# oneam/h264bsd

Hardware: AMD Instinct MI355X
Metric: 1080p macroblocks/s (higher is better)
Workload: dtype u8; 1 GPU; 256 concurrent copies of test_1920x1080.h264 per GPU (73 pictures x 8160 MB), kernel-only replay from HBM-resident frame jobs, inter+intra reconstruction + in-loop deblocking; streams_per_gpu=256, parallelism=streams/1, stream_groups=1, row_bands=library default (engine.hip TailConfig)

## Files before the change

h264bsd_amd/csrc/kernels/k_dbk.hip.h:

```cpp
#pragma once
namespace h264k {
#ifndef DBK_WGS
#define DBK_WGS 32
#endif
#ifndef DBK_WG_WAVES
#define DBK_WG_WAVES 4
#endif
__global__ __launch_bounds__(64 * DBK_WG_WAVES) void k_dbk(const FrameDesc *__restrict__ frames)
{
    __shared__ uint32_t s_tab[32 + 64];
    if (threadIdx.x < 64) {
        const uint32_t t = threadIdx.x, ok = t < 52;
        reinterpret_cast<uint8_t *>(s_tab)[t] = ok ? c_alpha[t] : 0;
        reinterpret_cast<uint8_t *>(s_tab)[64 + t] = ok ? c_beta[t] : 0;
        s_tab[32 + t] = ok ? (uint32_t)c_tc0[t][0] | ((uint32_t)c_tc0[t][1] << 8) | ((uint32_t)c_tc0[t][2] << 16) : 0u;
    }
    __syncthreads();
    const FrameDesc &fd = FD_REF(frames, blockIdx.y);
    const int m = threadIdx.x & 15;
    const int wmb = fd.wmb;
    const uint32_t n_dbk = fd.n_dbk;
    uint32_t di = blockIdx.x * (4 * DBK_WG_WAVES) + (threadIdx.x >> 4);
    const bool live0 = di < n_dbk;
    if (__ballot(live0) == 0ull) return;
    uint32_t mb = live0 ? fd.dbki[di] : 0u;
    bool live = live0;
  for (;;) {
    const uint32_t ndi = di + (4u * DBK_WG_WAVES) * gridDim.x;
    uint32_t nmb = mb;
    const bool nlive = live && ndi < n_dbk;
    if (nlive) nmb = fd.dbki[ndi];
    const uint32_t mbx = mb - mb_row(fd, mb) * (uint32_t)wmb;
    const uint32_t mbl = mbx ? mb - 1 : mb, mbt = mb >= (uint32_t)wmb ? mb - wmb : mb;
    FjMbRec q, pl, pt;
    const int dir = m >> 3, e = (m >> 1) & 3, kh = m & 1;
    int qx[2], qy[2], px[2], py[2];
    uint32_t mva[2], mvb[2];
#pragma unroll
    for (int kk = 0; kk < 2; kk++) {
        const int k = 2 * kh + kk;
        qx[kk] = dir ? k : e; qy[kk] = dir ? e : k;
        px[kk] = dir ? k : (e ? e - 1 : 3); py[kk] = dir ? (e ? e - 1 : 3) : k;
    }
    {
        const H264K_GLOBAL uint8_t *rq = (const H264K_GLOBAL uint8_t *)(fd.recs + mb), *rl = (const H264K_GLOBAL uint8_t *)(fd.recs + mbl),
                                   *rt = (const H264K_GLOBAL uint8_t *)(fd.recs + mbt);
        uint4 w[6] = { ld16g(rq), ld16g(rq + 16), ld16g(rl), ld16g(rl + 16), ld16g(rt), ld16g(rt + 16) };
#pragma unroll
        for (int i = 0; i < 6; i++) asm volatile("" : "+v"(w[i].x), "+v"(w[i].y), "+v"(w[i].z), "+v"(w[i].w));
        __builtin_memcpy(&q, &w[0], 32); __builtin_memcpy(&pl, &w[2], 32); __builtin_memcpy(&pt, &w[4], 32);
    }
    {
        const FjMbRec &pr = e ? q : (dir ? pt : pl);
        const bool q_one = (q.pred & FJ_PRED_UNIFORM_MV) || q.kind != FJ_MB_INTER, p_one = (pr.pred & FJ_PRED_UNIFORM_MV) || pr.kind != FJ_MB_INTER;
        const uint32_t q_mv = q.kind == FJ_MB_INTER ? (uint32_t)(uint16_t)q.mv[0] | ((uint32_t)(uint16_t)q.mv[1] << 16) : 0u;
        const uint32_t p_mv = pr.kind == FJ_MB_INTER ? (uint32_t)(uint16_t)pr.mv[0] | ((uint32_t)(uint16_t)pr.mv[1] << 16) : 0u;
#pragma unroll
        for (int kk = 0; kk < 2; kk++) {
            mva[kk] = q_mv; mvb[kk] = p_mv;
            if (!q_one) mva[kk] = *(const H264K_GLOBAL uint32_t *)(fd.mvx + 32 * (size_t)q.mvx + 2 * (4 * qy[kk] + qx[kk]));
            if (!p_one) mvb[kk] = *(const H264K_GLOBAL uint32_t *)(fd.mvx + 32 * (size_t)pr.mvx + 2 * (4 * py[kk] + px[kk]));
        }
    }
    uint8_t *out = fd.dbk + (size_t)mb * DBK_REC_BYTES;
    uint8_t *any_out = fd.dbk + (size_t)fd.n_mbs * DBK_REC_BYTES + mb;
    const bool filtered = live && q.dbk && q.kind != FJ_MB_ABSENT;
    if (live && !filtered && m == 0) { *reinterpret_cast<uint16_t *>(out + 46) = 0; *any_out = 0; }
    uint32_t bs2 = 0;
    const bool f_left = (q.dbk & FJ_DBK_LEFT) && mbx, f_top = (q.dbk & FJ_DBK_TOP) && mb >= (uint32_t)wmb;
    if (filtered) {
        const bool edge_on = e ? true : (dir ? f_top : f_left);
        if (edge_on) {
            const int p_kind = e ? q.kind : (dir ? pt.kind : pl.kind);
            const int parts = (q.pred >> FJ_PRED_PARTS_SHIFT) & 3;
            const uint32_t p_coded = e ? q.coded : (dir ? pt.coded : pl.coded);
            uint32_t qrefs, prefs, t0, t1;
            __builtin_memcpy(&qrefs, q.ref_slot, 4);
            __builtin_memcpy(&t0, pl.ref_slot, 4);
            __builtin_memcpy(&t1, pt.ref_slot, 4);
            prefs = e ? qrefs : (dir ? t1 : t0);
            const bool intra_edge = is_intra_kind(q.kind) || is_intra_kind(p_kind);
            const bool no_motion_edge = e && (parts == FJ_PARTS_16x16 || (parts == FJ_PARTS_16x8 && !(dir == 1 && e == 2)) || (parts == FJ_PARTS_8x16 && !(dir == 0 && e == 2)));
#pragma unroll
            for (int kk = 0; kk < 2; kk++) {
                int my_bs;
                if (intra_edge) my_bs = e ? 3 : 4;
                else if (((q.coded >> z_of(qx[kk], qy[kk])) & 1) || ((p_coded >> z_of(px[kk], py[kk])) & 1)) my_bs = 2;
                else if (no_motion_edge) my_bs = 0;
                else if (((qrefs >> (8 * ((qy[kk] >> 1) * 2 + (qx[kk] >> 1)))) & 255u) != ((prefs >> (8 * ((py[kk] >> 1) * 2 + (px[kk] >> 1)))) & 255u)) my_bs = 1;
                else {
                    const int ax = (int16_t)(mva[kk] & 0xFFFFu), ay = (int32_t)mva[kk] >> 16, bx2 = (int16_t)(mvb[kk] & 0xFFFFu), by2 = (int32_t)mvb[kk] >> 16;
                    my_bs = (abs(ax - bx2) >= 4 || abs(ay - by2) >= 4) ? 1 : 0;
                }
                bs2 |= (uint32_t)my_bs << (4 * kk);
            }
        }
    }
    uint32_t v = bs2;
    v |= (uint32_t)__builtin_amdgcn_update_dpp(0, (int)v, 0x101, 0xF, 0xF, true) << 8;
    v |= (uint32_t)__builtin_amdgcn_update_dpp(0, (int)v, 0x102, 0xF, 0xF, true) << 16;
    const unsigned long long bal = __ballot(bs2 != 0u);
    const uint32_t bal16 = (uint32_t)(bal >> (threadIdx.x & 48)) & 0xFFFFu;
    const bool any = bal16 != 0u;
    const uint32_t sched = (any ? DBKF_ANY : 0u) | ((bal16 & 0x0003u) ? DBKF_LEFT : 0u) | ((bal16 & 0x0300u) ? DBKF_TOP : 0u) |
                           ((bal16 & 0xFCFCu) ? DBKF_INNER : 0u);
    if (filtered) {
        if ((m & 3) == 0) *reinterpret_cast<uint32_t *>(out + m) = v;
        if (m < 6) {
            const int c = m;
            const int side = c % 3;
            const int pqp = side == 0 ? (int)pl.qp_y : side == 1 ? (int)pt.qp_y : (int)q.qp_y;
            int a = (int)q.qp_y, b = pqp;
            if (c >= 3) {
                a = qpc_of(clip3(0, 51, a + q.cqp_off));
                b = qpc_of(clip3(0, 51, b + q.cqp_off));
            }
            const int qpav = (a + b + 1) >> 1;
            const int ia = clip3(0, 51, qpav + q.alpha_off), ib = clip3(0, 51, qpav + q.beta_off);
            const uint32_t t = s_tab[32 + ia];
            *reinterpret_cast<uint32_t *>(out + 16 + 4 * c) = (uint32_t)reinterpret_cast<const uint8_t *>(s_tab)[ia] |
                ((uint32_t)reinterpret_cast<const uint8_t *>(s_tab)[64 + ib] << 8) | ((t & 0xFFFFu) << 16);
            out[40 + c] = (uint8_t)(t >> 16);
        }
        if (m == 12) {
            *reinterpret_cast<uint16_t *>(out + 46) = (uint16_t)((f_left ? FJ_DBK_LEFT : 0u) | (f_top ? FJ_DBK_TOP : 0u) | (q.dbk & FJ_DBK_INNER) | (any ? 0x100u : 0u));
            *any_out = (uint8_t)sched;
        }
    }
    if (__ballot(nlive) == 0ull) return;
    di = ndi; mb = nmb; live = nlive;
  }
}

}
```

Baseline: 1.782 billion macroblocks/s.

## Stage deblock MB records and output records through LDS with cooperative loads

Instead of every lane loading all three 32-byte macroblock records (current, left, top), six lanes per 16-lane group each load one 16-byte chunk into LDS. After a wave sync, each lane reads only the current record and the neighbour record it needs. The per-MB deblock output record is assembled in LDS and written back with three 16-byte stores in place of scattered 4-byte and byte stores. The default workgroup count per frame also doubles from 32 to 64. This cuts redundant global load traffic and VGPR pressure, at the cost of LDS use and extra wave syncs.

```diff
diff --git a/h264bsd_amd/csrc/kernels/k_dbk.hip.h b/h264bsd_amd/csrc/kernels/k_dbk.hip.h
--- a/h264bsd_amd/csrc/kernels/k_dbk.hip.h
+++ b/h264bsd_amd/csrc/kernels/k_dbk.hip.h
@@ -1,7 +1,7 @@
 #pragma once
 namespace h264k {
 #ifndef DBK_WGS
-#define DBK_WGS 32
+#define DBK_WGS 64
 #endif
 #ifndef DBK_WG_WAVES
 #define DBK_WG_WAVES 4
@@ -15,8 +15,12 @@
         reinterpret_cast<uint8_t *>(s_tab)[64 + t] = ok ? c_beta[t] : 0;
         s_tab[32 + t] = ok ? (uint32_t)c_tc0[t][0] | ((uint32_t)c_tc0[t][1] << 8) | ((uint32_t)c_tc0[t][2] << 16) : 0u;
     }
+    __shared__ u32x4 s_in[DBK_WG_WAVES][4][6];
+    __shared__ u32x4 s_out[DBK_WG_WAVES][4][3];
     __syncthreads();
     const FrameDesc &fd = FD_REF(frames, blockIdx.y);
+    H264K_LDS u32x4 *const in = (H264K_LDS u32x4 *)&s_in[threadIdx.x >> 6][(threadIdx.x >> 4) & 3][0];
+    H264K_LDS uint8_t *const rec = (H264K_LDS uint8_t *)&s_out[threadIdx.x >> 6][(threadIdx.x >> 4) & 3][0];
     const int m = threadIdx.x & 15;
     const int wmb = fd.wmb;
     const uint32_t n_dbk = fd.n_dbk;
@@ -32,7 +36,7 @@
     if (nlive) nmb = fd.dbki[ndi];
     const uint32_t mbx = mb - mb_row(fd, mb) * (uint32_t)wmb;
     const uint32_t mbl = mbx ? mb - 1 : mb, mbt = mb >= (uint32_t)wmb ? mb - wmb : mb;
-    FjMbRec q, pl, pt;
+    FjMbRec q, pr;
     const int dir = m >> 3, e = (m >> 1) & 3, kh = m & 1;
     int qx[2], qy[2], px[2], py[2];
     uint32_t mva[2], mvb[2];
@@ -42,16 +46,21 @@
         qx[kk] = dir ? k : e; qy[kk] = dir ? e : k;
         px[kk] = dir ? k : (e ? e - 1 : 3); py[kk] = dir ? (e ? e - 1 : 3) : k;
     }
+    const int side = m >= 3 ? m - 3 : m;
+    uint32_t pqp;
     {
-        const H264K_GLOBAL uint8_t *rq = (const H264K_GLOBAL uint8_t *)(fd.recs + mb), *rl = (const H264K_GLOBAL uint8_t *)(fd.recs + mbl),
-                                   *rt = (const H264K_GLOBAL uint8_t *)(fd.recs + mbt);
-        uint4 w[6] = { ld16g(rq), ld16g(rq + 16), ld16g(rl), ld16g(rl + 16), ld16g(rt), ld16g(rt + 16) };
-#pragma unroll
-        for (int i = 0; i < 6; i++) asm volatile("" : "+v"(w[i].x), "+v"(w[i].y), "+v"(w[i].z), "+v"(w[i].w));
-        __builtin_memcpy(&q, &w[0], 32); __builtin_memcpy(&pl, &w[2], 32); __builtin_memcpy(&pt, &w[4], 32);
+        if (m < 6) {
+            const uint32_t src = m < 2 ? mb : m < 4 ? mbl : mbt;
+            const uint4 w = ld16g((const H264K_GLOBAL uint8_t *)(fd.recs + src) + 16 * (m & 1));
+            in[m] = (u32x4){ w.x, w.y, w.z, w.w };
+        }
+        wave_sync();
+        const int pi = e ? 0 : dir ? 4 : 2;
+        const u32x4 w[4] = { in[0], in[1], in[pi], in[pi + 1] };
+        pqp = ((const H264K_LDS uint8_t *)(in + (side == 0 ? 2 : side == 1 ? 4 : 0)))[1];
+        __builtin_memcpy(&q, &w[0], 32); __builtin_memcpy(&pr, &w[2], 32);
     }
     {
-        const FjMbRec &pr = e ? q : (dir ? pt : pl);
         const bool q_one = (q.pred & FJ_PRED_UNIFORM_MV) || q.kind != FJ_MB_INTER, p_one = (pr.pred & FJ_PRED_UNIFORM_MV) || pr.kind != FJ_MB_INTER;
         const uint32_t q_mv = q.kind == FJ_MB_INTER ? (uint32_t)(uint16_t)q.mv[0] | ((uint32_t)(uint16_t)q.mv[1] << 16) : 0u;
         const uint32_t p_mv = pr.kind == FJ_MB_INTER ? (uint32_t)(uint16_t)pr.mv[0] | ((uint32_t)(uint16_t)pr.mv[1] << 16) : 0u;
@@ -62,23 +71,21 @@
             if (!p_one) mvb[kk] = *(const H264K_GLOBAL uint32_t *)(fd.mvx + 32 * (size_t)pr.mvx + 2 * (4 * py[kk] + px[kk]));
         }
     }
-    uint8_t *out = fd.dbk + (size_t)mb * DBK_REC_BYTES;
-    uint8_t *any_out = fd.dbk + (size_t)fd.n_mbs * DBK_REC_BYTES + mb;
+    H264K_GLOBAL uint8_t *out = (H264K_GLOBAL uint8_t *)fd.dbk + (size_t)mb * DBK_REC_BYTES;
+    H264K_GLOBAL uint8_t *any_out = (H264K_GLOBAL uint8_t *)fd.dbk + (size_t)fd.n_mbs * DBK_REC_BYTES + mb;
     const bool filtered = live && q.dbk && q.kind != FJ_MB_ABSENT;
-    if (live && !filtered && m == 0) { *reinterpret_cast<uint16_t *>(out + 46) = 0; *any_out = 0; }
+    if (live && !filtered && m == 0) *reinterpret_cast<H264K_GLOBAL uint16_t *>(out + 46) = 0;
     uint32_t bs2 = 0;
     const bool f_left = (q.dbk & FJ_DBK_LEFT) && mbx, f_top = (q.dbk & FJ_DBK_TOP) && mb >= (uint32_t)wmb;
     if (filtered) {
         const bool edge_on = e ? true : (dir ? f_top : f_left);
         if (edge_on) {
-            const int p_kind = e ? q.kind : (dir ? pt.kind : pl.kind);
+            const int p_kind = pr.kind;
             const int parts = (q.pred >> FJ_PRED_PARTS_SHIFT) & 3;
-            const uint32_t p_coded = e ? q.coded : (dir ? pt.coded : pl.coded);
-            uint32_t qrefs, prefs, t0, t1;
+            const uint32_t p_coded = pr.coded;
+            uint32_t qrefs, prefs;
             __builtin_memcpy(&qrefs, q.ref_slot, 4);
-            __builtin_memcpy(&t0, pl.ref_slot, 4);
-            __builtin_memcpy(&t1, pt.ref_slot, 4);
-            prefs = e ? qrefs : (dir ? t1 : t0);
+            __builtin_memcpy(&prefs, pr.ref_slot, 4);
             const bool intra_edge = is_intra_kind(q.kind) || is_intra_kind(p_kind);
             const bool no_motion_edge = e && (parts == FJ_PARTS_16x16 || (parts == FJ_PARTS_16x8 && !(dir == 1 && e == 2)) || (parts == FJ_PARTS_8x16 && !(dir == 0 && e == 2)));
 #pragma unroll
@@ -96,36 +103,33 @@
             }
         }
     }
-    uint32_t v = bs2;
-    v |= (uint32_t)__builtin_amdgcn_update_dpp(0, (int)v, 0x101, 0xF, 0xF, true) << 8;
-    v |= (uint32_t)__builtin_amdgcn_update_dpp(0, (int)v, 0x102, 0xF, 0xF, true) << 16;
     const unsigned long long bal = __ballot(bs2 != 0u);
     const uint32_t bal16 = (uint32_t)(bal >> (threadIdx.x & 48)) & 0xFFFFu;
     const bool any = bal16 != 0u;
     const uint32_t sched = (any ? DBKF_ANY : 0u) | ((bal16 & 0x0003u) ? DBKF_LEFT : 0u) | ((bal16 & 0x0300u) ? DBKF_TOP : 0u) |
                            ((bal16 & 0xFCFCu) ? DBKF_INNER : 0u);
-    if (filtered) {
-        if ((m & 3) == 0) *reinterpret_cast<uint32_t *>(out + m) = v;
-        if (m < 6) {
-            const int c = m;
-            const int side = c % 3;
-            const int pqp = side == 0 ? (int)pl.qp_y : side == 1 ? (int)pt.qp_y : (int)q.qp_y;
-            int a = (int)q.qp_y, b = pqp;
-            if (c >= 3) {
-                a = qpc_of(clip3(0, 51, a + q.cqp_off));
-                b = qpc_of(clip3(0, 51, b + q.cqp_off));
-            }
-            const int qpav = (a + b + 1) >> 1;
-            const int ia = clip3(0, 51, qpav + q.alpha_off), ib = clip3(0, 51, qpav + q.beta_off);
-            const uint32_t t = s_tab[32 + ia];
-            *reinterpret_cast<uint32_t *>(out + 16 + 4 * c) = (uint32_t)reinterpret_cast<const uint8_t *>(s_tab)[ia] |
-                ((uint32_t)reinterpret_cast<const uint8_t *>(s_tab)[64 + ib] << 8) | ((t & 0xFFFFu) << 16);
-            out[40 + c] = (uint8_t)(t >> 16);
+    if (live && m == 12) *any_out = (uint8_t)sched;
+    rec[m] = (uint8_t)bs2;
+    if (m < 6) {
+        const int c = m;
+        int a = (int)q.qp_y, b = (int)pqp;
+        if (c >= 3) {
+            a = qpc_of(clip3(0, 51, a + q.cqp_off));
+            b = qpc_of(clip3(0, 51, b + q.cqp_off));
         }
-        if (m == 12) {
-            *reinterpret_cast<uint16_t *>(out + 46) = (uint16_t)((f_left ? FJ_DBK_LEFT : 0u) | (f_top ? FJ_DBK_TOP : 0u) | (q.dbk & FJ_DBK_INNER) | (any ? 0x100u : 0u));
-            *any_out = (uint8_t)sched;
-        }
+        const int qpav = (a + b + 1) >> 1;
+        const int ia = clip3(0, 51, qpav + q.alpha_off), ib = clip3(0, 51, qpav + q.beta_off);
+        const uint32_t t = s_tab[32 + ia];
+        *reinterpret_cast<H264K_LDS uint32_t *>(rec + 16 + 4 * c) = (uint32_t)reinterpret_cast<const uint8_t *>(s_tab)[ia] |
+            ((uint32_t)reinterpret_cast<const uint8_t *>(s_tab)[64 + ib] << 8) | ((t & 0xFFFFu) << 16);
+        rec[40 + c] = (uint8_t)(t >> 16);
+    }
+    if (m == 12)
+        *reinterpret_cast<H264K_LDS uint16_t *>(rec + 46) = (uint16_t)((f_left ? FJ_DBK_LEFT : 0u) | (f_top ? FJ_DBK_TOP : 0u) | (q.dbk & FJ_DBK_INNER) | (any ? 0x100u : 0u));
+    wave_sync();
+    if (filtered && m < 3) {
+        const u32x4 w = reinterpret_cast<const H264K_LDS u32x4 *>(rec)[m];
+        st16g(out + 16 * m, make_uint4(w.x, w.y, w.z, w.w));
     }
     if (__ballot(nlive) == 0ull) return;
     di = ndi; mb = nmb; live = nlive;
```

Measured after the change: 1.789 billion macroblocks/s (median of 6 runs). Within noise of the previous version (+0.4%).
